# QEDProtocol/plonky2.5

Hardware: AMD Instinct MI355X
Metric: recursive proofs/sec (fib-64 p3-in-p2 circuit) (higher is better)
Workload: dtype u64 (Goldilocks, p = 2^64 - 2^32 + 1); 1 GPU; batch of 256 independent fib-64 plonky3-verifier proofs per GPU (n = 2^16 rows x 135 wires, LDE 2^19), 1 GPU(s), replicas + RCCL gather; all_statuses_ok=True, gathered_complete_and_ok=True, head=

## Files before the change

### plonky2.5_amd/csrc/poseidon.h

```cpp
#pragma once
#include "gl_lazy.h"

namespace poseidon {

constexpr int WIDTH = 12;
constexpr int RATE = 8;
constexpr int HALF_FULL = 4;
constexpr int N_PARTIAL = 22;
constexpr int N_ROUNDS = 30;

static constexpr u64 RC[360] = {
#include "poseidon_constants.inc"
};
static constexpr u32 MDS_CIRC[12] = {17, 15, 41, 16, 2, 28, 13, 13, 39, 18, 34, 20};
static constexpr u32 MDS_DIAG0 = 8;

GL_HD u64 sbox(u64 x) {
  u64 x2 = gl::mul_nc(x, x);
  u64 x4 = gl::mul_nc(x2, x2);
  u64 x3 = gl::mul_nc(x, x2);
  return gl::mul_nc(x3, x4);
}

GL_HD void mds(u64 s[WIDTH]) {
  u64 lo[WIDTH], hi[WIDTH];
#pragma unroll
  for (int i = 0; i < WIDTH; i++) {
    lo[i] = s[i] & gl::EPS;
    hi[i] = s[i] >> 32;
  }
#pragma unroll
  for (int r = 0; r < WIDTH; r++) {
    u64 al = 0, ah = 0;
#pragma unroll
    for (int i = 0; i < WIDTH; i++) {
      al += lo[(i + r) % WIDTH] * MDS_CIRC[i];
      ah += hi[(i + r) % WIDTH] * MDS_CIRC[i];
    }
    if (r == 0) {
      al += lo[0] * MDS_DIAG0;
      ah += hi[0] * MDS_DIAG0;
    }
    u64 l64 = al + (ah << 32);
    u32 h32 = (u32)(ah >> 32) + (l64 < al ? 1u : 0u);
    s[r] = gl::reduce96(l64, h32);
  }
}

GL_HD u64 add_rc(u64 x, u64 c) {
  u64 s = x + c;
  return s < x ? s + gl::EPS : s;
}

template <class Tracer>
GL_HD void permute_naive_trace(u64 s[WIDTH], Tracer&& tr) {
  int k = 0;
  for (int r = 0; r < N_ROUNDS; r++) {
    for (int i = 0; i < WIDTH; i++) s[i] = add_rc(s[i], RC[WIDTH * r + i]);
    if (r < HALF_FULL || r >= HALF_FULL + N_PARTIAL) {
      if (r != 0)
        for (int i = 0; i < WIDTH; i++) {
          s[i] = gl::canon(s[i]);
          tr(k++, s[i]);
        }
      for (int i = 0; i < WIDTH; i++) s[i] = sbox(s[i]);
    } else {
      s[0] = gl::canon(s[0]);
      tr(k++, s[0]);
      s[0] = sbox(s[0]);
    }
    mds(s);
  }
  for (int i = 0; i < WIDTH; i++) s[i] = gl::canon(s[i]);
}

#if defined(__HIP_DEVICE_COMPILE__)
struct RcSplit {
  u64 v[(N_ROUNDS + 1) * WIDTH * 2];
};
constexpr RcSplit make_rc_split() {
  RcSplit t{};
  for (int i = 0; i < N_ROUNDS * WIDTH; i++) {
    t.v[2 * i] = RC[i] & 0xFFFFFFFFull;
    t.v[2 * i + 1] = RC[i] >> 32;
  }
  return t;
}
static constexpr RcSplit RC_SPLIT = make_rc_split();

template <int C>
__device__ __forceinline__ void mad_k(u64& acc, u32 x) {
  u64 dm;
  asm("v_mad_u64_u32 %0, %1, %2, %3, %0" : "+v"(acc), "=s"(dm) : "v"(x), "n"(C));
}
typedef const u64 __attribute__((address_space(4))) * rc_ptr;
__device__ __forceinline__ void mds_rc(u64 s[WIDTH], rc_ptr k, u32 rows = 0xFFF) {
  u32 lo[WIDTH], hi[WIDTH];
#pragma unroll
  for (int i = 0; i < WIDTH; i++) {
    lo[i] = (u32)s[i];
    hi[i] = (u32)(s[i] >> 32);
  }
#pragma unroll
  for (int r = 0; r < WIDTH; r++) {
    if (!((rows >> r) & 1u)) continue;
    u64 al, ah, dm, t;
    asm("v_mad_u64_u32 %0, %1, %2, 17, %3" : "=v"(al), "=s"(dm) : "v"(lo[r]), "s"(k[2 * r]));
    asm("v_mad_u64_u32 %0, %1, %2, 17, %3" : "=v"(ah), "=s"(dm) : "v"(hi[r]), "s"(k[2 * r + 1]));
#define P25_MDS_TERM(i, C)            \
  mad_k<C>(al, lo[(i + r) % WIDTH]); \
  mad_k<C>(ah, hi[(i + r) % WIDTH]);
    P25_MDS_TERM(1, 15)
    P25_MDS_TERM(2, 41)
    P25_MDS_TERM(3, 16)
    P25_MDS_TERM(4, 2)
    P25_MDS_TERM(5, 28)
    P25_MDS_TERM(6, 13)
    P25_MDS_TERM(7, 13)
    P25_MDS_TERM(8, 39)
    P25_MDS_TERM(9, 18)
    P25_MDS_TERM(10, 34)
    P25_MDS_TERM(11, 20)
#undef P25_MDS_TERM
    if (r == 0) {
      mad_k<8>(al, lo[0]);
      mad_k<8>(ah, hi[0]);
    }
    u32 ahl = (u32)ah, ahh = (u32)(ah >> 32);
    u64 X;
    asm("v_mad_u64_u32 %0, %1, %2, -1, %3" : "=v"(X), "=s"(dm) : "v"(ahh), "v"(al));
    u32 x0 = (u32)X, x1 = (u32)(X >> 32);
    asm("v_add_co_u32_e32 %1, vcc, %1, %3\n\ts_nop 1\n\t"
        "v_subbrev_co_u32_e64 %0, %2, 0, %0, vcc\n\t"
        "s_andn2_b64 %2, vcc, %2\n\t"
        "v_addc_co_u32_e64 %1, %2, 0, %1, %2"
        : "+v"(x0), "+v"(x1), "=&s"(t)
        : "v"(ahl)
        : "vcc", "scc");
    s[r] = gl::make64(x0, x1);
  }
}
static_assert(MDS_CIRC[0] == 17 && MDS_CIRC[1] == 15 && MDS_CIRC[2] == 41 && MDS_CIRC[3] == 16 && MDS_CIRC[4] == 2 &&
                  MDS_CIRC[5] == 28 && MDS_CIRC[6] == 13 && MDS_CIRC[7] == 13 && MDS_CIRC[8] == 39 &&
                  MDS_CIRC[9] == 18 && MDS_CIRC[10] == 34 && MDS_CIRC[11] == 20 && MDS_DIAG0 == 8,
              "mds_rc hard-codes the MDS entries as inline constants");

#include "poseidon_p3r.h"

constexpr u64 sbox_const(u64 x) {
  const unsigned __int128 p = gl::P;
  u64 x2 = (u64)((unsigned __int128)x * x % p), x4 = (u64)((unsigned __int128)x2 * x2 % p), x3 = (u64)((unsigned __int128)x * x2 % p);
  return (u64)((unsigned __int128)x3 * x4 % p);
}
static constexpr u64 SBOX_RC0_CAP[4] = {sbox_const(RC[8]), sbox_const(RC[9]), sbox_const(RC[10]), sbox_const(RC[11])};

__device__ __forceinline__ void permute_dev(u64 s[WIDTH], u32 rows, bool cap0 = false) {
#pragma unroll
  for (int i = 0; i < RATE; i++) s[i] = add_rc(s[i], RC[i]);
  rc_ptr rc = (rc_ptr)RC_SPLIT.v;
  asm("" : "+s"(rc));
  int r = 1;
#pragma unroll
  for (int i = 0; i < RATE; i++) s[i] = sbox(s[i]);
  if (cap0) {
#pragma unroll
    for (int i = RATE; i < WIDTH; i++) s[i] = SBOX_RC0_CAP[i - RATE];
  } else {
#pragma unroll
    for (int i = RATE; i < WIDTH; i++) s[i] = sbox(add_rc(s[i], RC[i]));
  }
  mds_rc(s, rc + 2 * WIDTH * r);
  r++;
  for (int k = 1; k < HALF_FULL - 1; k++, r++) {
#pragma unroll
    for (int i = 0; i < WIDTH; i++) s[i] = sbox(s[i]);
    mds_rc(s, rc + 2 * WIDTH * r);
  }
#pragma unroll
  for (int i = 0; i < WIDTH; i++) s[i] = sbox(s[i]);
  p3r::tbl_ptr tp = (p3r::tbl_ptr)&p3r::TBL;
  asm("" : "+s"(tp));
  p3r::three_rounds<true>(s, tp, tp->kh);
  for (int b = 0; b < p3r::BLOCKS; b++) p3r::three_rounds<false>(s, tp, tp->kc[b]);
  p3r::two_rounds(s, tp);
  r = HALF_FULL + N_PARTIAL + 1;
  for (int k = 0; k < HALF_FULL - 1; k++, r++) {
#pragma unroll
    for (int i = 0; i < WIDTH; i++) s[i] = sbox(s[i]);
    mds_rc(s, rc + 2 * WIDTH * r);
  }
#pragma unroll
  for (int i = 0; i < WIDTH; i++) s[i] = sbox(s[i]);
  mds_rc(s, rc + 2 * WIDTH * N_ROUNDS, rows);
#pragma unroll
  for (int i = 0; i < WIDTH; i++) s[i] = gl::canon(s[i]);
}
#endif

GL_HD void permute_rows(u64 s[WIDTH], u32 rows, bool cap0 = false) {
#if defined(__HIP_DEVICE_COMPILE__)
  permute_dev(s, rows, cap0);
#else
  (void)rows;
  (void)cap0;
  int r = 0;
  for (int k = 0; k < HALF_FULL; k++, r++) {
#pragma unroll
    for (int i = 0; i < WIDTH; i++) s[i] = sbox(add_rc(s[i], RC[12 * r + i]));
    mds(s);
  }
  for (int k = 0; k < N_PARTIAL; k++, r++) {
#pragma unroll
    for (int i = 0; i < WIDTH; i++) s[i] = add_rc(s[i], RC[12 * r + i]);
    s[0] = sbox(s[0]);
    mds(s);
  }
  for (int k = 0; k < HALF_FULL; k++, r++) {
#pragma unroll
    for (int i = 0; i < WIDTH; i++) s[i] = sbox(add_rc(s[i], RC[12 * r + i]));
    mds(s);
  }
#pragma unroll
  for (int i = 0; i < WIDTH; i++) s[i] = gl::canon(s[i]);
#endif
}

GL_HD void permute(u64 s[WIDTH]) { permute_rows(s, 0xFFF); }
constexpr u32 ROWS_DIGEST = 0x00F, ROWS_CAPACITY = 0xF00, ROWS_ALL = 0xFFF;

GL_HD void two_to_one(const u64 l[4], const u64 r[4], u64 out[4]) {
  u64 s[WIDTH];
#pragma unroll
  for (int i = 0; i < 4; i++) {
    s[i] = l[i];
    s[4 + i] = r[i];
    s[8 + i] = 0;
  }
  permute_rows(s, ROWS_DIGEST, true);
#pragma unroll
  for (int i = 0; i < 4; i++) out[i] = s[i];
}

GL_HD void hash_no_pad_strided(const u64* in, size_t stride, int n, u64 out[4]) {
  u64 s[WIDTH];
#pragma unroll
  for (int i = 0; i < WIDTH; i++) s[i] = 0;
  for (int off = 0; off < n; off += RATE) {
    int m = n - off < RATE ? n - off : RATE;
    for (int i = 0; i < m; i++) s[i] = in[(size_t)(off + i) * stride];
    const int next = n - (off + RATE);
    permute_rows(s, next <= 0 ? ROWS_DIGEST : (next >= RATE ? ROWS_CAPACITY : ROWS_ALL), off == 0);
  }
#pragma unroll
  for (int i = 0; i < 4; i++) out[i] = s[i];
}

GL_HD void hash_or_noop_strided(const u64* in, size_t stride, int n, u64 out[4]) {
  if (n <= 4) {
    for (int i = 0; i < 4; i++) out[i] = i < n ? in[(size_t)i * stride] : 0;
  } else {
    hash_no_pad_strided(in, stride, n, out);
  }
}

}
```

### plonky2.5_amd/csrc/poseidon_p3r.h

```cpp
#pragma once

namespace p3r {

constexpr int BLOCKS = 6;
constexpr int HEAD_ROUND = 3;
constexpr int FIRST_BLOCK = 6;
constexpr int TAIL_ROUND = 24;
static_assert(HEAD_ROUND == HALF_FULL - 1 && FIRST_BLOCK + 3 * BLOCKS == TAIL_ROUND &&
                  TAIL_ROUND + 2 == HALF_FULL + N_PARTIAL,
              "partial-round schedule");

struct Row16 {
  u32 c[16];
};
struct Tables {
  Row16 t3[WIDTH];
  Row16 t2[WIDTH];
  Row16 r2;
  u32 kc[BLOCKS][64];
  u32 kh[64];
  u32 kt[64];
};

constexpr u64 mulmod(u64 a, u64 b) { return (u64)((unsigned __int128)a * b % gl::P); }
constexpr u64 addmod(u64 a, u64 b) { return (u64)(((unsigned __int128)a + b) % gl::P); }
constexpr u64 mds_entry(int r, int j) { return MDS_CIRC[(j - r + WIDTH) % WIDTH] + (r == 0 && j == 0 ? MDS_DIAG0 : 0); }

constexpr void block_constants(u32* out, int r0, const u64 (&M)[WIDTH][WIDTH], const u64 (&M2)[WIDTH][WIDTH],
                               const u64 (&M3)[WIDTH][WIDTH], u64 (&o)[WIDTH]) {
  const u64* c1 = RC + WIDTH * (r0 + 1);
  const u64* c2 = RC + WIDTH * (r0 + 2);
  const u64* c3 = RC + WIDTH * (r0 + 3);
  u64 k1 = c1[0];
  u64 k2 = c2[0];
  for (int j = 0; j < WIDTH; j++) {
    k1 = addmod(k1, mulmod(M[0][j], o[j]));
    k2 = addmod(k2, addmod(mulmod(M[0][j], c1[j]), mulmod(M2[0][j], o[j])));
  }
  out[0] = (u32)k1;
  out[1] = (u32)(k1 >> 32);
  out[2] = (u32)k2;
  out[3] = (u32)(k2 >> 32);
  u64 on[WIDTH] = {};
  for (int r = 0; r < WIDTH; r++) {
    u64 k3 = c3[r];
    for (int j = 0; j < WIDTH; j++)
      k3 = addmod(k3, addmod(addmod(mulmod(M2[r][j], c1[j]), mulmod(M[r][j], c2[j])), mulmod(M3[r][j], o[j])));
    on[r] = k3;
  }
  out[4] = (u32)on[0];
  out[5] = (u32)(on[0] >> 32);
  for (int r = 1; r < WIDTH; r++) {
    out[4 + 2 * r] = 0;
    out[5 + 2 * r] = 0;
  }
  on[0] = 0;
  for (int r = 0; r < WIDTH; r++) o[r] = on[r];
}

constexpr Tables make_tables() {
  Tables t{};
  u64 M[WIDTH][WIDTH] = {}, M2[WIDTH][WIDTH] = {}, M3[WIDTH][WIDTH] = {};
  for (int r = 0; r < WIDTH; r++)
    for (int j = 0; j < WIDTH; j++) M[r][j] = mds_entry(r, j);
  for (int r = 0; r < WIDTH; r++)
    for (int j = 0; j < WIDTH; j++)
      for (int k = 0; k < WIDTH; k++) M2[r][j] += M[r][k] * M[k][j];
  for (int r = 0; r < WIDTH; r++)
    for (int j = 0; j < WIDTH; j++)
      for (int k = 0; k < WIDTH; k++) M3[r][j] += M2[r][k] * M[k][j];
  for (int r = 0; r < WIDTH; r++) {
    for (int j = 0; j < WIDTH; j++) {
      t.t3[r].c[j] = (u32)M3[r][j];
      t.t2[r].c[j] = (u32)M2[r][j];
    }
    t.t3[r].c[12] = (u32)M3[r][0];
    t.t3[r].c[13] = (u32)M2[r][0];
    t.t3[r].c[14] = (u32)M[r][0];
    t.t2[r].c[12] = (u32)M2[r][0];
    t.t2[r].c[13] = (u32)M[r][0];
  }
  for (int j = 0; j < WIDTH; j++) t.r2.c[j] = (u32)M2[0][j];
  t.r2.c[12] = (u32)M2[0][0];
  t.r2.c[13] = (u32)M[0][0];
  u64 o[WIDTH] = {};
  block_constants(t.kh, HEAD_ROUND, M, M2, M3, o);
  for (int b = 0; b < BLOCKS; b++) block_constants(t.kc[b], FIRST_BLOCK + 3 * b, M, M2, M3, o);
  {
    const u64* c1 = RC + WIDTH * (TAIL_ROUND + 1);
    const u64* c2 = RC + WIDTH * (TAIL_ROUND + 2);
    u64 k1 = c1[0];
    for (int j = 0; j < WIDTH; j++) k1 = addmod(k1, mulmod(M[0][j], o[j]));
    t.kt[0] = (u32)k1;
    t.kt[1] = (u32)(k1 >> 32);
    for (int r = 0; r < WIDTH; r++) {
      u64 k = c2[r];
      for (int j = 0; j < WIDTH; j++) k = addmod(k, addmod(mulmod(M[r][j], c1[j]), mulmod(M2[r][j], o[j])));
      t.kt[4 + 2 * r] = (u32)k;
      t.kt[5 + 2 * r] = (u32)(k >> 32);
    }
  }
  return t;
}
static constexpr Tables TBL = make_tables();

constexpr u64 sbox_ref(u64 x) {
  u64 x2 = mulmod(x, x), x4 = mulmod(x2, x2), x3 = mulmod(x, x2);
  return mulmod(x3, x4);
}
constexpr u64 kpair(const u32* k, int i) { return (u64)k[i] | ((u64)k[i + 1] << 32); }
constexpr void rounds_ref(u64 (&w)[WIDTH], int r0, int n, bool skip_first) {
  for (int k = 0; k < n; k++) {
    u64 y[WIDTH] = {};
    for (int i = 0; i < WIDTH; i++) y[i] = w[i];
    if (!(skip_first && k == 0)) y[0] = sbox_ref(y[0]);
    for (int r = 0; r < WIDTH; r++) {
      u64 acc = RC[WIDTH * (r0 + k + 1) + r];
      for (int j = 0; j < WIDTH; j++) acc = addmod(acc, mulmod(mds_entry(r, j), y[j]));
      w[r] = acc;
    }
  }
}
constexpr void block_emulated(u64 (&v)[WIDTH], const u32* kc, bool skip_first) {
  u64 d[3] = {};
  u64 x = v[0];
  d[0] = skip_first ? 0 : addmod(sbox_ref(x), gl::P - x);
  u64 a = kpair(kc, 0);
  for (int j = 0; j < WIDTH; j++) a = addmod(a, mulmod(mds_entry(0, j), v[j]));
  a = addmod(a, mulmod(mds_entry(0, 0), d[0]));
  x = a;
  d[1] = addmod(sbox_ref(x), gl::P - x);
  a = kpair(kc, 2);
  for (int j = 0; j < WIDTH; j++) a = addmod(a, mulmod(TBL.r2.c[j], v[j]));
  a = addmod(a, addmod(mulmod(TBL.r2.c[12], d[0]), mulmod(TBL.r2.c[13], d[1])));
  x = a;
  d[2] = addmod(sbox_ref(x), gl::P - x);
  u64 w[WIDTH] = {};
  for (int r = 0; r < WIDTH; r++) {
    a = r == 0 ? kpair(kc, 4) : 0;
    for (int j = 0; j < WIDTH; j++) a = addmod(a, mulmod(TBL.t3[r].c[j], v[j]));
    for (int e = 0; e < 3; e++) a = addmod(a, mulmod(TBL.t3[r].c[12 + e], d[e]));
    w[r] = a;
  }
  for (int r = 0; r < WIDTH; r++) v[r] = w[r];
}
constexpr void tail_emulated(u64 (&v)[WIDTH]) {
  u64 d[2] = {};
  u64 x = v[0];
  d[0] = addmod(sbox_ref(x), gl::P - x);
  u64 a = kpair(TBL.kt, 0);
  for (int j = 0; j < WIDTH; j++) a = addmod(a, mulmod(mds_entry(0, j), v[j]));
  a = addmod(a, mulmod(mds_entry(0, 0), d[0]));
  x = a;
  d[1] = addmod(sbox_ref(x), gl::P - x);
  u64 w[WIDTH] = {};
  for (int r = 0; r < WIDTH; r++) {
    a = kpair(TBL.kt, 4 + 2 * r);
    for (int j = 0; j < WIDTH; j++) a = addmod(a, mulmod(TBL.t2[r].c[j], v[j]));
    for (int e = 0; e < 2; e++) a = addmod(a, mulmod(TBL.t2[r].c[12 + e], d[e]));
    w[r] = a;
  }
  for (int r = 0; r < WIDTH; r++) v[r] = w[r];
}
constexpr bool chain_consistent(int salt) {
  u64 v[WIDTH] = {}, w[WIDTH] = {};
  for (int i = 0; i < WIDTH; i++) v[i] = w[i] = mulmod(0x9E3779B97F4A7C15ull % gl::P, (u64)(i + 1 + 13 * salt));
  rounds_ref(w, HEAD_ROUND, 3, true);
  for (int b = 0; b < BLOCKS; b++) rounds_ref(w, FIRST_BLOCK + 3 * b, 3, false);
  rounds_ref(w, TAIL_ROUND, 2, false);
  block_emulated(v, TBL.kh, true);
  for (int b = 0; b < BLOCKS; b++) block_emulated(v, TBL.kc[b], false);
  tail_emulated(v);
  for (int r = 0; r < WIDTH; r++)
    if (v[r] != w[r]) return false;
  return true;
}
constexpr bool tables_consistent() { return chain_consistent(0) && chain_consistent(7) && chain_consistent(101); }
static_assert(tables_consistent(), "poseidon_p3r.h: block tables disagree with the round-by-round definition");

typedef const Tables __attribute__((address_space(4))) * tbl_ptr;
typedef const u32 __attribute__((address_space(4))) * k_ptr;

__device__ __forceinline__ void mad_s(u64& acc, u32 x, u32 coef_sgpr) {
  u64 dm;
  asm("v_mad_u64_u32 %0, %1, %2, %3, %0" : "+v"(acc), "=s"(dm) : "v"(x), "s"(coef_sgpr));
}
__device__ __forceinline__ u64 mul_s(u32 x, u32 coef_sgpr) {
  u64 acc, dm;
  asm("v_mad_u64_u32 %0, %1, %2, %3, 0" : "=v"(acc), "=s"(dm) : "v"(x), "s"(coef_sgpr));
  return acc;
}
__device__ __forceinline__ void add_s(u64& acc, u32 k_sgpr) {
  u64 dm;
  asm("v_mad_u64_u32 %0, %1, 1, %2, %0" : "+v"(acc), "=s"(dm) : "s"(k_sgpr));
}
__device__ __forceinline__ u64 reduce_row(u64 al, u64 ah) {
  u32 ahl = (u32)ah, ahh = (u32)(ah >> 32);
  u64 X, dm, t;
  asm("v_mad_u64_u32 %0, %1, %2, -1, %3" : "=v"(X), "=s"(dm) : "v"(ahh), "v"(al));
  u32 x0 = (u32)X, x1 = (u32)(X >> 32);
  asm("v_add_co_u32_e32 %1, vcc, %1, %3\n\ts_nop 1\n\t"
      "v_subbrev_co_u32_e64 %0, %2, 0, %0, vcc\n\t"
      "s_andn2_b64 %2, vcc, %2\n\t"
      "v_addc_co_u32_e64 %1, %2, 0, %1, %2"
      : "+v"(x0), "+v"(x1), "=&s"(t)
      : "v"(ahl)
      : "vcc", "scc");
  return gl::make64(x0, x1);
}

template <int E0, int NEXTRA, bool WITH_K = true>
__device__ __forceinline__ u64 row(const u32* lo, const u32* hi, const Row16& cf, const u32* dlo, const u32* dhi,
                                   u32 klo, u32 khi) {
  u64 al = mul_s(lo[0], cf.c[0]), ah = mul_s(hi[0], cf.c[0]);
#pragma unroll
  for (int j = 1; j < WIDTH; j++) {
    mad_s(al, lo[j], cf.c[j]);
    mad_s(ah, hi[j], cf.c[j]);
  }
#pragma unroll
  for (int e = E0; e < E0 + NEXTRA; e++) {
    mad_s(al, dlo[e], cf.c[12 + e]);
    mad_s(ah, dhi[e], cf.c[12 + e]);
  }
  if (WITH_K) {
    add_s(al, klo);
    add_s(ah, khi);
  }
  return reduce_row(al, ah);
}
template <bool WITH_D>
__device__ __forceinline__ u64 row0_m(const u32* lo, const u32* hi, u32 dlo, u32 dhi, u32 klo, u32 khi) {
  u64 al = 0, ah = 0;
  mad_k<25>(al, lo[0]);  mad_k<25>(ah, hi[0]);
  mad_k<15>(al, lo[1]);  mad_k<15>(ah, hi[1]);
  mad_k<41>(al, lo[2]);  mad_k<41>(ah, hi[2]);
  mad_k<16>(al, lo[3]);  mad_k<16>(ah, hi[3]);
  mad_k<2>(al, lo[4]);   mad_k<2>(ah, hi[4]);
  mad_k<28>(al, lo[5]);  mad_k<28>(ah, hi[5]);
  mad_k<13>(al, lo[6]);  mad_k<13>(ah, hi[6]);
  mad_k<13>(al, lo[7]);  mad_k<13>(ah, hi[7]);
  mad_k<39>(al, lo[8]);  mad_k<39>(ah, hi[8]);
  mad_k<18>(al, lo[9]);  mad_k<18>(ah, hi[9]);
  mad_k<34>(al, lo[10]); mad_k<34>(ah, hi[10]);
  mad_k<20>(al, lo[11]); mad_k<20>(ah, hi[11]);
  if (WITH_D) {
    mad_k<25>(al, dlo);
    mad_k<25>(ah, dhi);
  }
  add_s(al, klo);
  add_s(ah, khi);
  return reduce_row(al, ah);
}
__device__ __forceinline__ void load_row(Row16& cf, const Row16 __attribute__((address_space(4))) * src) {
#pragma unroll
  for (int j = 0; j < 16; j++) cf.c[j] = src->c[j];
}
__device__ __forceinline__ void delta(u64 x, u32& dlo, u32& dhi) {
  const u64 d = gl::sub_nc(sbox(x), x);
  dlo = (u32)d;
  dhi = (u32)(d >> 32);
}

template <bool HEAD>
__device__ __forceinline__ void three_rounds(u64 s[WIDTH], tbl_ptr tp, k_ptr kc) {
  u32 lo[WIDTH], hi[WIDTH];
#pragma unroll
  for (int i = 0; i < WIDTH; i++) {
    lo[i] = (u32)s[i];
    hi[i] = (u32)(s[i] >> 32);
  }
  u32 dlo[3] = {0, 0, 0}, dhi[3] = {0, 0, 0};
  if (!HEAD) delta(s[0], dlo[0], dhi[0]);
  u64 x = row0_m<!HEAD>(lo, hi, dlo[0], dhi[0], kc[0], kc[1]);
  delta(x, dlo[1], dhi[1]);
  {
    Row16 cf;
    load_row(cf, &tp->r2);
    x = row<HEAD ? 1 : 0, HEAD ? 1 : 2>(lo, hi, cf, dlo, dhi, kc[2], kc[3]);
  }
  delta(x, dlo[2], dhi[2]);
#pragma unroll
  for (int r = 0; r < WIDTH; r++) {
    Row16 cf;
    load_row(cf, &tp->t3[r]);
    if (r == 0)
      s[r] = row<HEAD ? 1 : 0, HEAD ? 2 : 3, true>(lo, hi, cf, dlo, dhi, kc[4], kc[5]);
    else
      s[r] = row<HEAD ? 1 : 0, HEAD ? 2 : 3, false>(lo, hi, cf, dlo, dhi, 0, 0);
  }
}
__device__ __forceinline__ void two_rounds(u64 s[WIDTH], tbl_ptr tp) {
  u32 lo[WIDTH], hi[WIDTH];
#pragma unroll
  for (int i = 0; i < WIDTH; i++) {
    lo[i] = (u32)s[i];
    hi[i] = (u32)(s[i] >> 32);
  }
  const k_ptr kc = tp->kt;
  u32 dlo[2], dhi[2];
  delta(s[0], dlo[0], dhi[0]);
  const u64 x = row0_m<true>(lo, hi, dlo[0], dhi[0], kc[0], kc[1]);
  delta(x, dlo[1], dhi[1]);
#pragma unroll
  for (int r = 0; r < WIDTH; r++) {
    Row16 cf;
    load_row(cf, &tp->t2[r]);
    s[r] = row<0, 2>(lo, hi, cf, dlo, dhi, kc[4 + 2 * r], kc[5 + 2 * r]);
  }
}

}
```

Baseline: 138.0 proofs/s.

## Batch Poseidon partial rounds into four-round blocks with precomputed MDS powers

Restructures the partial-round fast path. It moves from a head, six three-round blocks and a two-round tail to a head plus five four-round blocks that apply precomputed M^4 rows. A shared-sum term keeps the coefficients within 32 bits. The MDS diagonal is folded into the first multiply-add, and hash_no_pad skips output rows that are overwritten by the next absorb. The goal is fewer MDS multiply-adds and reductions per permutation, at the cost of larger coefficient tables and more intricate constexpr correctness checks.

```diff
diff --git a/plonky2.5_amd/csrc/poseidon.h b/plonky2.5_amd/csrc/poseidon.h
--- a/plonky2.5_amd/csrc/poseidon.h
+++ b/plonky2.5_amd/csrc/poseidon.h
@@ -105,8 +105,13 @@
   for (int r = 0; r < WIDTH; r++) {
     if (!((rows >> r) & 1u)) continue;
     u64 al, ah, dm, t;
-    asm("v_mad_u64_u32 %0, %1, %2, 17, %3" : "=v"(al), "=s"(dm) : "v"(lo[r]), "s"(k[2 * r]));
-    asm("v_mad_u64_u32 %0, %1, %2, 17, %3" : "=v"(ah), "=s"(dm) : "v"(hi[r]), "s"(k[2 * r + 1]));
+    if (r == 0) {
+      asm("v_mad_u64_u32 %0, %1, %2, 25, %3" : "=v"(al), "=s"(dm) : "v"(lo[r]), "s"(k[2 * r]));
+      asm("v_mad_u64_u32 %0, %1, %2, 25, %3" : "=v"(ah), "=s"(dm) : "v"(hi[r]), "s"(k[2 * r + 1]));
+    } else {
+      asm("v_mad_u64_u32 %0, %1, %2, 17, %3" : "=v"(al), "=s"(dm) : "v"(lo[r]), "s"(k[2 * r]));
+      asm("v_mad_u64_u32 %0, %1, %2, 17, %3" : "=v"(ah), "=s"(dm) : "v"(hi[r]), "s"(k[2 * r + 1]));
+    }
 #define P25_MDS_TERM(i, C)            \
   mad_k<C>(al, lo[(i + r) % WIDTH]); \
   mad_k<C>(ah, hi[(i + r) % WIDTH]);
@@ -122,10 +127,6 @@
     P25_MDS_TERM(10, 34)
     P25_MDS_TERM(11, 20)
 #undef P25_MDS_TERM
-    if (r == 0) {
-      mad_k<8>(al, lo[0]);
-      mad_k<8>(ah, hi[0]);
-    }
     u32 ahl = (u32)ah, ahh = (u32)(ah >> 32);
     u64 X;
     asm("v_mad_u64_u32 %0, %1, %2, -1, %3" : "=v"(X), "=s"(dm) : "v"(ahh), "v"(al));
@@ -145,8 +146,11 @@
                   MDS_CIRC[9] == 18 && MDS_CIRC[10] == 34 && MDS_CIRC[11] == 20 && MDS_DIAG0 == 8,
               "mds_rc hard-codes the MDS entries as inline constants");
 
+#endif
+
 #include "poseidon_p3r.h"
 
+#if defined(__HIP_DEVICE_COMPILE__)
 constexpr u64 sbox_const(u64 x) {
   const unsigned __int128 p = gl::P;
   u64 x2 = (u64)((unsigned __int128)x * x % p), x4 = (u64)((unsigned __int128)x2 * x2 % p), x3 = (u64)((unsigned __int128)x * x2 % p);
@@ -178,11 +182,7 @@
   }
 #pragma unroll
   for (int i = 0; i < WIDTH; i++) s[i] = sbox(s[i]);
-  p3r::tbl_ptr tp = (p3r::tbl_ptr)&p3r::TBL;
-  asm("" : "+s"(tp));
-  p3r::three_rounds<true>(s, tp, tp->kh);
-  for (int b = 0; b < p3r::BLOCKS; b++) p3r::three_rounds<false>(s, tp, tp->kc[b]);
-  p3r::two_rounds(s, tp);
+  p3r::partial_rounds(s);
   r = HALF_FULL + N_PARTIAL + 1;
   for (int k = 0; k < HALF_FULL - 1; k++, r++) {
 #pragma unroll
@@ -249,7 +249,7 @@
     int m = n - off < RATE ? n - off : RATE;
     for (int i = 0; i < m; i++) s[i] = in[(size_t)(off + i) * stride];
     const int next = n - (off + RATE);
-    permute_rows(s, next <= 0 ? ROWS_DIGEST : (next >= RATE ? ROWS_CAPACITY : ROWS_ALL), off == 0);
+    permute_rows(s, next <= 0 ? ROWS_DIGEST : (next >= RATE ? ROWS_CAPACITY : ROWS_ALL & ~((1u << next) - 1u)), off == 0);
   }
 #pragma unroll
   for (int i = 0; i < 4; i++) out[i] = s[i];
diff --git a/plonky2.5_amd/csrc/poseidon_p3r.h b/plonky2.5_amd/csrc/poseidon_p3r.h
--- a/plonky2.5_amd/csrc/poseidon_p3r.h
+++ b/plonky2.5_amd/csrc/poseidon_p3r.h
@@ -2,107 +2,112 @@
 
 namespace p3r {
 
-constexpr int BLOCKS = 6;
+constexpr int BLOCKS = 5;
 constexpr int HEAD_ROUND = 3;
 constexpr int FIRST_BLOCK = 6;
-constexpr int TAIL_ROUND = 24;
-static_assert(HEAD_ROUND == HALF_FULL - 1 && FIRST_BLOCK + 3 * BLOCKS == TAIL_ROUND &&
-                  TAIL_ROUND + 2 == HALF_FULL + N_PARTIAL,
+static_assert(HEAD_ROUND == HALF_FULL - 1 && FIRST_BLOCK == HEAD_ROUND + 3 &&
+                  FIRST_BLOCK + 4 * BLOCKS == HALF_FULL + N_PARTIAL,
               "partial-round schedule");
+constexpr int SHIFT4 = 28;
 
 struct Row16 {
   u32 c[16];
 };
 struct Tables {
   Row16 t3[WIDTH];
-  Row16 t2[WIDTH];
+  Row16 t4[WIDTH];
   Row16 r2;
-  u32 kc[BLOCKS][64];
-  u32 kh[64];
-  u32 kt[64];
+  u32 kh[32];
+  u32 kc[BLOCKS][32];
+  u64 off[BLOCKS + 1][WIDTH];
+};
+struct Powers {
+  u64 m[5][WIDTH][WIDTH];
 };
 
 constexpr u64 mulmod(u64 a, u64 b) { return (u64)((unsigned __int128)a * b % gl::P); }
 constexpr u64 addmod(u64 a, u64 b) { return (u64)(((unsigned __int128)a + b) % gl::P); }
 constexpr u64 mds_entry(int r, int j) { return MDS_CIRC[(j - r + WIDTH) % WIDTH] + (r == 0 && j == 0 ? MDS_DIAG0 : 0); }
 
-constexpr void block_constants(u32* out, int r0, const u64 (&M)[WIDTH][WIDTH], const u64 (&M2)[WIDTH][WIDTH],
-                               const u64 (&M3)[WIDTH][WIDTH], u64 (&o)[WIDTH]) {
-  const u64* c1 = RC + WIDTH * (r0 + 1);
-  const u64* c2 = RC + WIDTH * (r0 + 2);
-  const u64* c3 = RC + WIDTH * (r0 + 3);
-  u64 k1 = c1[0];
-  u64 k2 = c2[0];
-  for (int j = 0; j < WIDTH; j++) {
-    k1 = addmod(k1, mulmod(M[0][j], o[j]));
-    k2 = addmod(k2, addmod(mulmod(M[0][j], c1[j]), mulmod(M2[0][j], o[j])));
-  }
-  out[0] = (u32)k1;
-  out[1] = (u32)(k1 >> 32);
-  out[2] = (u32)k2;
-  out[3] = (u32)(k2 >> 32);
-  u64 on[WIDTH] = {};
-  for (int r = 0; r < WIDTH; r++) {
-    u64 k3 = c3[r];
-    for (int j = 0; j < WIDTH; j++)
-      k3 = addmod(k3, addmod(addmod(mulmod(M2[r][j], c1[j]), mulmod(M[r][j], c2[j])), mulmod(M3[r][j], o[j])));
-    on[r] = k3;
-  }
-  out[4] = (u32)on[0];
-  out[5] = (u32)(on[0] >> 32);
-  for (int r = 1; r < WIDTH; r++) {
-    out[4 + 2 * r] = 0;
-    out[5 + 2 * r] = 0;
-  }
-  on[0] = 0;
-  for (int r = 0; r < WIDTH; r++) o[r] = on[r];
+constexpr Powers make_powers() {
+  Powers p{};
+  for (int r = 0; r < WIDTH; r++) {
+    p.m[0][r][r] = 1;
+    for (int j = 0; j < WIDTH; j++) p.m[1][r][j] = mds_entry(r, j);
+  }
+  for (int e = 2; e <= 4; e++)
+    for (int r = 0; r < WIDTH; r++)
+      for (int j = 0; j < WIDTH; j++)
+        for (int k = 0; k < WIDTH; k++) p.m[e][r][j] += p.m[e - 1][r][k] * p.m[1][k][j];
+  return p;
+}
+
+constexpr void block_constants(u32* out, int r0, int n, const Powers& p, u64 (&o)[WIDTH], bool last) {
+  u64 oc[WIDTH] = {};
+  for (int j = 0; j < WIDTH; j++) oc[j] = o[j];
+  for (int i = 1; i <= n; i++) {
+    for (int r = 0; r < (i < n ? 1 : WIDTH); r++) {
+      u64 k = RC[WIDTH * (r0 + i) + r];
+      for (int j = 0; j < WIDTH; j++) {
+        for (int m = 1; m < i; m++) k = addmod(k, mulmod(p.m[m][r][j], RC[WIDTH * (r0 + i - m) + j]));
+        k = addmod(k, mulmod(p.m[i][r][j], oc[j]));
+      }
+      const int at = 2 * (i - 1) + 2 * r;
+      const bool now = i < n || r == 0 || last;
+      out[at] = now ? (u32)k : 0;
+      out[at + 1] = now ? (u32)(k >> 32) : 0;
+      if (i == n) o[r] = now ? 0 : k;
+    }
+  }
 }
 
 constexpr Tables make_tables() {
   Tables t{};
-  u64 M[WIDTH][WIDTH] = {}, M2[WIDTH][WIDTH] = {}, M3[WIDTH][WIDTH] = {};
-  for (int r = 0; r < WIDTH; r++)
-    for (int j = 0; j < WIDTH; j++) M[r][j] = mds_entry(r, j);
-  for (int r = 0; r < WIDTH; r++)
+  const Powers p = make_powers();
+  for (int r = 0; r < WIDTH; r++) {
+    for (int j = 0; j < WIDTH; j++) {
+      t.t3[r].c[j] = (u32)p.m[3][r][j];
+      t.t4[r].c[j] = (u32)(p.m[4][r][j] - ((u64)1 << SHIFT4));
+    }
+    t.t3[r].c[13] = (u32)p.m[2][r][0];
+    t.t3[r].c[14] = (u32)p.m[1][r][0];
+    t.t4[r].c[12] = 1u << SHIFT4;
+    t.t4[r].c[13] = (u32)p.m[3][r][0];
+    t.t4[r].c[14] = (u32)p.m[2][r][0];
+    t.t4[r].c[15] = (u32)p.m[1][r][0];
+  }
+  for (int j = 0; j < WIDTH; j++) t.r2.c[j] = (u32)p.m[2][0][j];
+  t.r2.c[13] = (u32)p.m[1][0][0];
+  u64 o[WIDTH] = {};
+  block_constants(t.kh, HEAD_ROUND, 3, p, o, false);
+  for (int b = 0; b < BLOCKS; b++) {
+    for (int r = 0; r < WIDTH; r++) t.off[b][r] = o[r];
+    block_constants(t.kc[b], FIRST_BLOCK + 4 * b, 4, p, o, b == BLOCKS - 1);
+  }
+  for (int r = 0; r < WIDTH; r++) t.off[BLOCKS][r] = o[r];
+  return t;
+}
+static constexpr Tables TBL = make_tables();
+
+constexpr bool fits63(const Row16& cf, int e0, int nextra) {
+  u64 sum = 1;
+  for (int j = 0; j < WIDTH; j++) sum += cf.c[j];
+  for (int e = e0; e < e0 + nextra; e++) sum += cf.c[12 + e];
+  return (unsigned __int128)sum * 0xFFFFFFFFu < ((unsigned __int128)1 << 63);
+}
+constexpr bool rows_carry_free() {
+  const Powers p = make_powers();
+  Row16 m0{};
+  for (int j = 0; j < WIDTH; j++) m0.c[j] = (u32)mds_entry(0, j);
+  bool ok = fits63(m0, 0, 0) && fits63(TBL.r2, 1, 1);
+  for (int r = 0; r < WIDTH; r++) {
+    ok = ok && fits63(TBL.t3[r], 1, 2) && fits63(TBL.t4[r], 0, 4);
     for (int j = 0; j < WIDTH; j++)
-      for (int k = 0; k < WIDTH; k++) M2[r][j] += M[r][k] * M[k][j];
-  for (int r = 0; r < WIDTH; r++)
-    for (int j = 0; j < WIDTH; j++)
-      for (int k = 0; k < WIDTH; k++) M3[r][j] += M2[r][k] * M[k][j];
-  for (int r = 0; r < WIDTH; r++) {
-    for (int j = 0; j < WIDTH; j++) {
-      t.t3[r].c[j] = (u32)M3[r][j];
-      t.t2[r].c[j] = (u32)M2[r][j];
-    }
-    t.t3[r].c[12] = (u32)M3[r][0];
-    t.t3[r].c[13] = (u32)M2[r][0];
-    t.t3[r].c[14] = (u32)M[r][0];
-    t.t2[r].c[12] = (u32)M2[r][0];
-    t.t2[r].c[13] = (u32)M[r][0];
-  }
-  for (int j = 0; j < WIDTH; j++) t.r2.c[j] = (u32)M2[0][j];
-  t.r2.c[12] = (u32)M2[0][0];
-  t.r2.c[13] = (u32)M[0][0];
-  u64 o[WIDTH] = {};
-  block_constants(t.kh, HEAD_ROUND, M, M2, M3, o);
-  for (int b = 0; b < BLOCKS; b++) block_constants(t.kc[b], FIRST_BLOCK + 3 * b, M, M2, M3, o);
-  {
-    const u64* c1 = RC + WIDTH * (TAIL_ROUND + 1);
-    const u64* c2 = RC + WIDTH * (TAIL_ROUND + 2);
-    u64 k1 = c1[0];
-    for (int j = 0; j < WIDTH; j++) k1 = addmod(k1, mulmod(M[0][j], o[j]));
-    t.kt[0] = (u32)k1;
-    t.kt[1] = (u32)(k1 >> 32);
-    for (int r = 0; r < WIDTH; r++) {
-      u64 k = c2[r];
-      for (int j = 0; j < WIDTH; j++) k = addmod(k, addmod(mulmod(M[r][j], c1[j]), mulmod(M2[r][j], o[j])));
-      t.kt[4 + 2 * r] = (u32)k;
-      t.kt[5 + 2 * r] = (u32)(k >> 32);
-    }
-  }
-  return t;
-}
-static constexpr Tables TBL = make_tables();
+      ok = ok && p.m[4][r][j] >= ((u64)1 << SHIFT4) && p.m[4][r][j] - ((u64)1 << SHIFT4) <= 0xFFFFFFFFu;
+  }
+  return ok;
+}
+static_assert(rows_carry_free(), "poseidon_p3r.h: a row accumulator can reach 2^63");
 
 constexpr u64 sbox_ref(u64 x) {
   u64 x2 = mulmod(x, x), x4 = mulmod(x2, x2), x3 = mulmod(x, x2);
@@ -121,56 +126,68 @@
     }
   }
 }
-constexpr void block_emulated(u64 (&v)[WIDTH], const u32* kc, bool skip_first) {
-  u64 d[3] = {};
-  u64 x = v[0];
-  d[0] = skip_first ? 0 : addmod(sbox_ref(x), gl::P - x);
-  u64 a = kpair(kc, 0);
-  for (int j = 0; j < WIDTH; j++) a = addmod(a, mulmod(mds_entry(0, j), v[j]));
-  a = addmod(a, mulmod(mds_entry(0, 0), d[0]));
-  x = a;
-  d[1] = addmod(sbox_ref(x), gl::P - x);
-  a = kpair(kc, 2);
-  for (int j = 0; j < WIDTH; j++) a = addmod(a, mulmod(TBL.r2.c[j], v[j]));
-  a = addmod(a, addmod(mulmod(TBL.r2.c[12], d[0]), mulmod(TBL.r2.c[13], d[1])));
-  x = a;
-  d[2] = addmod(sbox_ref(x), gl::P - x);
+constexpr u64 halves_value(unsigned __int128 al, unsigned __int128 ah) {
+  return (u64)((al % gl::P + (ah % gl::P << 32)) % gl::P);
+}
+constexpr bool row_emulated(u64& out, const u64 (&v)[WIDTH], const Row16& cf, const u64 (&d)[4], int e0, int nextra,
+                            u64 k) {
+  unsigned __int128 al = (u32)k, ah = k >> 32;
+  for (int j = 0; j < WIDTH; j++) {
+    al += (unsigned __int128)cf.c[j] * (u32)v[j];
+    ah += (unsigned __int128)cf.c[j] * (v[j] >> 32);
+  }
+  for (int e = e0; e < e0 + nextra; e++) {
+    al += (unsigned __int128)cf.c[12 + e] * (u32)d[e];
+    ah += (unsigned __int128)cf.c[12 + e] * (d[e] >> 32);
+  }
+  out = halves_value(al, ah);
+  return (al >> 63) == 0 && (ah >> 63) == 0;
+}
+constexpr u64 delta_ref(u64 x) { return addmod(sbox_ref(x), gl::P - x % gl::P); }
+constexpr bool block_emulated(u64 (&v)[WIDTH], const u32* kc, bool four, bool last) {
+  Row16 m0{};
+  for (int j = 0; j < WIDTH; j++) m0.c[j] = (u32)mds_entry(0, j);
+  u64 d[4] = {};
+  u64 x = 0;
+  bool ok = true;
+  if (four) v[0] = sbox_ref(v[0]);
+  ok = row_emulated(x, v, m0, d, 0, 0, kpair(kc, 0)) && ok;
+  d[1] = delta_ref(x);
+  ok = row_emulated(x, v, TBL.r2, d, 1, 1, kpair(kc, 2)) && ok;
+  d[2] = delta_ref(x);
+  if (four) {
+    ok = row_emulated(x, v, TBL.t3[0], d, 1, 2, kpair(kc, 4)) && ok;
+    d[3] = delta_ref(x);
+    unsigned __int128 ul = 0, uh = 0;
+    for (int j = 0; j < WIDTH; j++) {
+      ul += (u32)v[j];
+      uh += v[j] >> 32;
+    }
+    d[0] = halves_value(ul, uh);
+  }
   u64 w[WIDTH] = {};
   for (int r = 0; r < WIDTH; r++) {
-    a = r == 0 ? kpair(kc, 4) : 0;
-    for (int j = 0; j < WIDTH; j++) a = addmod(a, mulmod(TBL.t3[r].c[j], v[j]));
-    for (int e = 0; e < 3; e++) a = addmod(a, mulmod(TBL.t3[r].c[12 + e], d[e]));
-    w[r] = a;
+    const u64 k = (r == 0 || last) ? kpair(kc, (four ? 6 : 4) + 2 * r) : 0;
+    ok = (four ? row_emulated(w[r], v, TBL.t4[r], d, 0, 4, k) : row_emulated(w[r], v, TBL.t3[r], d, 1, 2, k)) && ok;
   }
   for (int r = 0; r < WIDTH; r++) v[r] = w[r];
-}
-constexpr void tail_emulated(u64 (&v)[WIDTH]) {
-  u64 d[2] = {};
-  u64 x = v[0];
-  d[0] = addmod(sbox_ref(x), gl::P - x);
-  u64 a = kpair(TBL.kt, 0);
-  for (int j = 0; j < WIDTH; j++) a = addmod(a, mulmod(mds_entry(0, j), v[j]));
-  a = addmod(a, mulmod(mds_entry(0, 0), d[0]));
-  x = a;
-  d[1] = addmod(sbox_ref(x), gl::P - x);
-  u64 w[WIDTH] = {};
-  for (int r = 0; r < WIDTH; r++) {
-    a = kpair(TBL.kt, 4 + 2 * r);
-    for (int j = 0; j < WIDTH; j++) a = addmod(a, mulmod(TBL.t2[r].c[j], v[j]));
-    for (int e = 0; e < 2; e++) a = addmod(a, mulmod(TBL.t2[r].c[12 + e], d[e]));
-    w[r] = a;
-  }
-  for (int r = 0; r < WIDTH; r++) v[r] = w[r];
+  return ok;
+}
+constexpr void chain_ref(u64 (&w)[WIDTH]) {
+  for (int i = 0; i < WIDTH; i++) w[i] %= gl::P;
+  rounds_ref(w, HEAD_ROUND, 3, true);
+  rounds_ref(w, FIRST_BLOCK, 4 * BLOCKS, false);
+}
+constexpr bool chain_emulated(u64 (&v)[WIDTH]) {
+  bool ok = block_emulated(v, TBL.kh, false, false);
+  for (int b = 0; b < BLOCKS; b++) ok = block_emulated(v, TBL.kc[b], true, b == BLOCKS - 1) && ok;
+  return ok;
 }
 constexpr bool chain_consistent(int salt) {
   u64 v[WIDTH] = {}, w[WIDTH] = {};
   for (int i = 0; i < WIDTH; i++) v[i] = w[i] = mulmod(0x9E3779B97F4A7C15ull % gl::P, (u64)(i + 1 + 13 * salt));
-  rounds_ref(w, HEAD_ROUND, 3, true);
-  for (int b = 0; b < BLOCKS; b++) rounds_ref(w, FIRST_BLOCK + 3 * b, 3, false);
-  rounds_ref(w, TAIL_ROUND, 2, false);
-  block_emulated(v, TBL.kh, true);
-  for (int b = 0; b < BLOCKS; b++) block_emulated(v, TBL.kc[b], false);
-  tail_emulated(v);
+  chain_ref(w);
+  if (!chain_emulated(v)) return false;
   for (int r = 0; r < WIDTH; r++)
     if (v[r] != w[r]) return false;
   return true;
@@ -178,6 +195,7 @@
 constexpr bool tables_consistent() { return chain_consistent(0) && chain_consistent(7) && chain_consistent(101); }
 static_assert(tables_consistent(), "poseidon_p3r.h: block tables disagree with the round-by-round definition");
 
+#if defined(__HIP_DEVICE_COMPILE__)
 typedef const Tables __attribute__((address_space(4))) * tbl_ptr;
 typedef const u32 __attribute__((address_space(4))) * k_ptr;
 
@@ -188,6 +206,12 @@
 __device__ __forceinline__ u64 mul_s(u32 x, u32 coef_sgpr) {
   u64 acc, dm;
   asm("v_mad_u64_u32 %0, %1, %2, %3, 0" : "=v"(acc), "=s"(dm) : "v"(x), "s"(coef_sgpr));
+  return acc;
+}
+template <int C>
+__device__ __forceinline__ u64 mul_k(u32 x) {
+  u64 acc, dm;
+  asm("v_mad_u64_u32 %0, %1, %2, %3, 0" : "=v"(acc), "=s"(dm) : "v"(x), "n"(C));
   return acc;
 }
 __device__ __forceinline__ void add_s(u64& acc, u32 k_sgpr) {
@@ -229,10 +253,8 @@
   }
   return reduce_row(al, ah);
 }
-template <bool WITH_D>
-__device__ __forceinline__ u64 row0_m(const u32* lo, const u32* hi, u32 dlo, u32 dhi, u32 klo, u32 khi) {
-  u64 al = 0, ah = 0;
-  mad_k<25>(al, lo[0]);  mad_k<25>(ah, hi[0]);
+__device__ __forceinline__ u64 row0_m(const u32* lo, const u32* hi, u32 klo, u32 khi) {
+  u64 al = mul_k<25>(lo[0]), ah = mul_k<25>(hi[0]);
   mad_k<15>(al, lo[1]);  mad_k<15>(ah, hi[1]);
   mad_k<41>(al, lo[2]);  mad_k<41>(ah, hi[2]);
   mad_k<16>(al, lo[3]);  mad_k<16>(ah, hi[3]);
@@ -244,12 +266,17 @@
   mad_k<18>(al, lo[9]);  mad_k<18>(ah, hi[9]);
   mad_k<34>(al, lo[10]); mad_k<34>(ah, hi[10]);
   mad_k<20>(al, lo[11]); mad_k<20>(ah, hi[11]);
-  if (WITH_D) {
-    mad_k<25>(al, dlo);
-    mad_k<25>(ah, dhi);
-  }
   add_s(al, klo);
   add_s(ah, khi);
+  return reduce_row(al, ah);
+}
+__device__ __forceinline__ u64 shared_sum(const u32* lo, const u32* hi) {
+  u64 al = mul_k<1>(lo[0]), ah = mul_k<1>(hi[0]);
+#pragma unroll
+  for (int j = 1; j < WIDTH; j++) {
+    mad_k<1>(al, lo[j]);
+    mad_k<1>(ah, hi[j]);
+  }
   return reduce_row(al, ah);
 }
 __device__ __forceinline__ void load_row(Row16& cf, const Row16 __attribute__((address_space(4))) * src) {
@@ -261,23 +288,24 @@
   dlo = (u32)d;
   dhi = (u32)(d >> 32);
 }
-
-template <bool HEAD>
-__device__ __forceinline__ void three_rounds(u64 s[WIDTH], tbl_ptr tp, k_ptr kc) {
-  u32 lo[WIDTH], hi[WIDTH];
+__device__ __forceinline__ void split(const u64 s[WIDTH], u32 lo[WIDTH], u32 hi[WIDTH]) {
 #pragma unroll
   for (int i = 0; i < WIDTH; i++) {
     lo[i] = (u32)s[i];
     hi[i] = (u32)(s[i] >> 32);
   }
-  u32 dlo[3] = {0, 0, 0}, dhi[3] = {0, 0, 0};
-  if (!HEAD) delta(s[0], dlo[0], dhi[0]);
-  u64 x = row0_m<!HEAD>(lo, hi, dlo[0], dhi[0], kc[0], kc[1]);
+}
+
+__device__ __forceinline__ void head_block(u64 s[WIDTH], tbl_ptr tp, k_ptr kc) {
+  u32 lo[WIDTH], hi[WIDTH];
+  split(s, lo, hi);
+  u32 dlo[3], dhi[3];
+  u64 x = row0_m(lo, hi, kc[0], kc[1]);
   delta(x, dlo[1], dhi[1]);
   {
     Row16 cf;
     load_row(cf, &tp->r2);
-    x = row<HEAD ? 1 : 0, HEAD ? 1 : 2>(lo, hi, cf, dlo, dhi, kc[2], kc[3]);
+    x = row<1, 1>(lo, hi, cf, dlo, dhi, kc[2], kc[3]);
   }
   delta(x, dlo[2], dhi[2]);
 #pragma unroll
@@ -285,29 +313,51 @@
     Row16 cf;
     load_row(cf, &tp->t3[r]);
     if (r == 0)
-      s[r] = row<HEAD ? 1 : 0, HEAD ? 2 : 3, true>(lo, hi, cf, dlo, dhi, kc[4], kc[5]);
+      s[r] = row<1, 2, true>(lo, hi, cf, dlo, dhi, kc[4], kc[5]);
     else
-      s[r] = row<HEAD ? 1 : 0, HEAD ? 2 : 3, false>(lo, hi, cf, dlo, dhi, 0, 0);
-  }
-}
-__device__ __forceinline__ void two_rounds(u64 s[WIDTH], tbl_ptr tp) {
+      s[r] = row<1, 2, false>(lo, hi, cf, dlo, dhi, 0, 0);
+  }
+}
+__device__ __forceinline__ void four_rounds(u64 s[WIDTH], tbl_ptr tp, k_ptr kc, bool last) {
+  s[0] = sbox(s[0]);
   u32 lo[WIDTH], hi[WIDTH];
-#pragma unroll
-  for (int i = 0; i < WIDTH; i++) {
-    lo[i] = (u32)s[i];
-    hi[i] = (u32)(s[i] >> 32);
-  }
-  const k_ptr kc = tp->kt;
-  u32 dlo[2], dhi[2];
-  delta(s[0], dlo[0], dhi[0]);
-  const u64 x = row0_m<true>(lo, hi, dlo[0], dhi[0], kc[0], kc[1]);
+  split(s, lo, hi);
+  u32 dlo[4], dhi[4];
+  u64 x = row0_m(lo, hi, kc[0], kc[1]);
   delta(x, dlo[1], dhi[1]);
-#pragma unroll
-  for (int r = 0; r < WIDTH; r++) {
-    Row16 cf;
-    load_row(cf, &tp->t2[r]);
-    s[r] = row<0, 2>(lo, hi, cf, dlo, dhi, kc[4 + 2 * r], kc[5 + 2 * r]);
-  }
-}
-
-}
+  {
+    Row16 cf;
+    load_row(cf, &tp->r2);
+    x = row<1, 1>(lo, hi, cf, dlo, dhi, kc[2], kc[3]);
+  }
+  delta(x, dlo[2], dhi[2]);
+  {
+    Row16 cf;
+    load_row(cf, &tp->t3[0]);
+    x = row<1, 2>(lo, hi, cf, dlo, dhi, kc[4], kc[5]);
+  }
+  delta(x, dlo[3], dhi[3]);
+  {
+    const u64 u = shared_sum(lo, hi);
+    dlo[0] = (u32)u;
+    dhi[0] = (u32)(u >> 32);
+  }
+#pragma unroll
+  for (int r = 0; r < WIDTH; r++) {
+    Row16 cf;
+    load_row(cf, &tp->t4[r]);
+    if (r == 0 || last)
+      s[r] = row<0, 4, true>(lo, hi, cf, dlo, dhi, kc[6 + 2 * r], kc[7 + 2 * r]);
+    else
+      s[r] = row<0, 4, false>(lo, hi, cf, dlo, dhi, 0, 0);
+  }
+}
+__device__ __forceinline__ void partial_rounds(u64 s[WIDTH]) {
+  tbl_ptr tp = (tbl_ptr)&TBL;
+  asm("" : "+s"(tp));
+  head_block(s, tp, tp->kh);
+  for (int b = 0; b < BLOCKS; b++) four_rounds(s, tp, tp->kc[b], b == BLOCKS - 1);
+}
+#endif
+
+}
```

Measured after the change: 141.6 proofs/s, median of 6. +2.6%, better.
